# corywalker/llm_inference

Hardware: AMD Instinct MI355X
Metric: decode tokens/sec + achieved HBM GB/s vs roofline, Gemma-3 4B Q4_0 (higher is better)
Workload: dtype q4_0 x q8_0 int8 dot, fp32 accumulate; f16 logits table; 1 GPU; gemma-3-4b-q4_0 greedy decode after a 512-token prefill (BASELINE configs[2]); mode=fast, parallelism=single

## Files before the change

include/llmi.h:

```cpp
#ifndef LLMI_H
#define LLMI_H

#include <stddef.h>
#include <stdint.h>

#ifdef __cplusplus
extern "C" {
#endif

typedef enum {
  LLMI_OK = 0,
  LLMI_E_SIZE = 1,
  LLMI_E_TYPE = 2,
  LLMI_E_ARG = 3,
  LLMI_E_HIP = 4,
  LLMI_E_GGUF = 5,
  LLMI_E_NODEV = 6,
  LLMI_E_RANGE = 7
} llmi_status;

#define LLMI_EXACT 1u
#define LLMI_NO_GRAPH 2u
#define LLMI_TP_PEER 4u
#define LLMI_EXACT_KQ 8u
// ... 113 lines not shown

int llmi_session_enqueue(llmi_session* s, int32_t first, int pos, int n_steps);
int llmi_session_sync(llmi_session* s, int32_t* out_tokens, int n);

typedef struct {
  int n_layer, n_embd, n_ff, n_head, n_head_kv, head_dim, vocab, max_ctx;
  size_t weight_bytes;
  size_t bytes_per_token;
  size_t kv_bytes_per_pos;
  int kernels_per_token;
  int tp_rank, tp_size;
  int batched_prefill;
  int screened_logits;
  size_t screen_bytes;
  int prefill_f16_redo;
  int layer_engine;
  int ffn_engine;
  int tp_exchange;
  long long block_slow_waits;
  int exact_engine;
  int exact_batched_prefill;
  int prefill_gemm;
  int sampling;
  int score_path;
} llmi_session_info;
#define LLMI_SESSION_INFO_N_SEQ_OFFSET 132
#define LLMI_SESSION_INFO_N_SEQ(info) (*(const int*)((const char*)(info) + LLMI_SESSION_INFO_N_SEQ_OFFSET))
int llmi_session_get_info_sized(const llmi_session* s, llmi_session_info* info, size_t info_size);
int llmi_session_get_info(const llmi_session* s, llmi_session_info* info);
#define llmi_session_get_info(s, info) llmi_session_get_info_sized((s), (info), sizeof(llmi_session_info))

int llmi_session_time_kernel(llmi_session* s, int which, int reps, double* us_per_launch, double* bytes_per_launch);

int llmi_selftest(int which, unsigned long long* out);

#ifdef __cplusplus
}
#endif
#endif
```

llm_inference_amd/_lib.py:

```python
from __future__ import annotations

import ctypes as C
import os

import numpy as np

HERE = os.path.dirname(os.path.abspath(__file__))
LIB_PATH = os.environ.get("LLMI_LIB") or os.path.join(HERE, "libllmi.so")

LLMI_EXACT = 1
LLMI_NO_GRAPH = 2
LLMI_TP_PEER = 4
LLMI_EXACT_KQ = 8
PEER_HANDLE_BYTES = 64

STATUS = {0: "OK", 1: "E_SIZE", 2: "E_TYPE", 3: "E_ARG", 4: "E_HIP", 5: "E_GGUF", 6: "E_NODEV", 7: "E_RANGE"}


class LLMIError(RuntimeError):

    def __init__(self, code: int, msg: str):
        super().__init__(msg)
        self.code = code
        self.status = STATUS.get(code, str(code))
# ... 78 lines not shown
    "llmi_session_create":(C.c_int, [_vp, _sz, C.POINTER(SessionOpts), C.POINTER(_vp)]),
    "llmi_session_destroy": (None, [_vp]),
    "llmi_tp_unique_id": (C.c_int, [_vp]),
    "llmi_tp_group_create": (C.c_int, [C.c_int, C.POINTER(_vp)]),
    "llmi_tp_group_destroy": (None, [_vp]),
    "llmi_session_peer_handle": (C.c_int, [_vp, _vp]),
    "llmi_session_peer_connect": (C.c_int, [_vp, _vp]),
    "llmi_session_forward": (C.c_int, [_vp, _vp, C.c_int, C.c_int, _vp, _vp]),
    "llmi_session_score": (C.c_int, [_vp, _vp, C.c_int, C.c_int, _vp, _vp, _vp, _vp]),
    "llmi_session_seq_reserve": (C.c_int, [_vp, C.c_int]),
    "llmi_session_seq_copy": (C.c_int, [_vp, C.c_int, C.c_int, C.c_int]),
    "llmi_session_batch_forward": (C.c_int, [_vp, _vp, _vp, _vp, C.c_int, _vp, _vp, _vp]),
    "llmi_session_batch_extend": (C.c_int, [_vp, _vp, C.POINTER(Span), C.c_int, _vp, _vp, _vp]),
    "llmi_session_batch_generate": (C.c_int, [_vp, _vp, _vp, _vp, C.c_int, C.c_int, _vp, C.c_int, _vp]),
    "llmi_session_batch_generate_sampled": (C.c_int, [_vp, _vp, _vp, _vp, C.c_int, C.c_int, _vp, C.c_int,
                                                      C.POINTER(Sampler), _vp]),
    "llmi_session_batch_generate_lookup": (C.c_int, [_vp, _vp, _vp, _vp, _vp, C.c_int, C.POINTER(Lookup), C.c_int, _vp,
                                                     C.c_int, _vp, _vp, C.POINTER(LookupStats)]),
    "llmi_lookup_draft": (C.c_int, [_vp, C.c_int, C.c_int, C.c_int, C.c_int, _vp, C.POINTER(C.c_int),
                                    C.POINTER(C.c_int), C.POINTER(C.c_int)]),
    "llmi_logits_rows": (C.c_int, [_vp, _vp, C.c_int, C.c_int, C.c_int, _f32, _vp]),
    "llmi_logits_rows_rb": (C.c_int, [C.c_int]),
    "llmi_score_rows": (C.c_int, [_vp, _vp, C.c_int, C.c_int, C.c_int, _f32, _vp, _vp, _vp, _vp]),
    "llmi_session_generate": (C.c_int, [_vp, _i32, C.c_int, C.c_int, _vp]),
    "llmi_session_dump": (C.c_int, [_vp, _vp, C.c_int, C.c_int, C.c_char_p]),
    "llmi_session_enqueue": (C.c_int, [_vp, _i32, C.c_int, C.c_int]),
    "llmi_session_trace": (C.c_int, [_vp, _vp, C.c_int, C.c_int, _u32, _vp, _vp]),
    "llmi_session_sync": (C.c_int, [_vp, _vp, C.c_int]),
    "llmi_session_set_sampler": (C.c_int, [_vp, C.POINTER(Sampler)]),
    "llmi_sample_logits": (C.c_int, [_vp, _sz, C.POINTER(Sampler), C.c_int, _vp, _vp, _vp, _vp, _vp]),
    "llmi_session_get_info": (C.c_int, [_vp, _vp]),
    "llmi_session_get_info_sized": (C.c_int, [_vp, C.POINTER(SessionInfo), _sz]),
    "llmi_session_time_kernel": (C.c_int, [_vp, C.c_int, C.c_int, C.POINTER(_f64), C.POINTER(_f64)]),
    "llmi_selftest": (C.c_int, [C.c_int, _vp]),
}


def lib() -> C.CDLL:
    global _lib
    if _lib is None:
        if not os.path.exists(LIB_PATH):
            raise ImportError(f"{LIB_PATH} missing: build it with `python -m llm_inference_amd.build` "
                              "(HIP, --offload-arch=gfx950); there is no CPU fallback")
        L = C.CDLL(LIB_PATH)
        for name, (res, args) in _SIGS.items():
            f = getattr(L, name)
            f.restype = res
            f.argtypes = args
        _lib = L
    return _lib


def check(rc: int) -> None:
    if rc != 0:
        raise LLMIError(rc, lib().llmi_last_error().decode(errors="replace"))


def ptr(a: np.ndarray) -> int:
    return a.ctypes.data
```

llm_inference_amd/csrc/capi.cpp:

```cpp
#include <algorithm>
#include <cmath>
#include <cstddef>
#include <cstring>
#include <mutex>
#include <vector>

#include "score_plan.h"
#include "session.h"

using namespace llmi;

namespace {

thread_local std::string g_err;

struct Ctx {
  int device = -1;
  hipStream_t stream = nullptr;
  hipEvent_t ev_in = nullptr, ev_out = nullptr;
  std::vector<std::pair<void*, size_t>> bufs;
  void* get(int slot, size_t bytes) {
    if ((int)bufs.size() <= slot) bufs.resize(slot + 1, {nullptr, 0});
    auto& b = bufs[slot];
    if (b.second < bytes) {
// ... 701 lines not shown
      out[1] = r[1];
    } else if (which == 2) {
      size_t live = 0, cached = 0, grave = 0;
      dev_mem_stats(&live, &cached, &grave);
      out[0] = live;
      out[1] = cached;
      out[2] = grave;
    } else {
      throw status_error(LLMI_E_ARG, "selftest: unknown test");
    }
  });
}

int llmi_session_get_info_sized(const llmi_session* s, llmi_session_info* info, size_t info_size) {
  return guard([&] {
    if (!s || !info) throw status_error(LLMI_E_ARG, "get_info: null pointer");
    llmi_session_info full;
    std::memset(&full, 0, sizeof(full));
    s->s->info(&full);
    static_assert(sizeof(llmi_session_info) == LLMI_SESSION_INFO_N_SEQ_OFFSET + sizeof(int) &&
                      offsetof(llmi_session_info, score_path) + sizeof(int) == LLMI_SESSION_INFO_N_SEQ_OFFSET,
                  "n_seq lies in llmi_session_info's tail padding");
    const int n_seq = s->s->n_seq();
    std::memcpy(reinterpret_cast<char*>(&full) + LLMI_SESSION_INFO_N_SEQ_OFFSET, &n_seq, sizeof(int));
    std::memcpy(info, &full, std::min(info_size, sizeof(full)));
  });
}

static_assert(offsetof(llmi_session_info, score_path) == 128, "the struct's layout before score_path was appended");
int (llmi_session_get_info)(const llmi_session* s, llmi_session_info* info) {
  return llmi_session_get_info_sized(s, info, offsetof(llmi_session_info, score_path));
}

int llmi_session_time_kernel(llmi_session* s, int which, int reps, double* us, double* bytes) {
  return guard([&] { s->s->time_kernel(which, reps, us, bytes); });
}

}
```

llm_inference_amd/csrc/k_logits.hip:

```cpp
#include "session_kernels.h"

namespace llmi {

namespace {

__device__ __forceinline__ float dot8_h(uint4 w, uint4 x, float acc) {
  typedef _Float16 h2t __attribute__((ext_vector_type(2)));
  acc = __builtin_amdgcn_fdot2(__builtin_bit_cast(h2t, w.x), __builtin_bit_cast(h2t, x.x), acc, false);
  acc = __builtin_amdgcn_fdot2(__builtin_bit_cast(h2t, w.y), __builtin_bit_cast(h2t, x.y), acc, false);
  acc = __builtin_amdgcn_fdot2(__builtin_bit_cast(h2t, w.z), __builtin_bit_cast(h2t, x.z), acc, false);
  acc = __builtin_amdgcn_fdot2(__builtin_bit_cast(h2t, w.w), __builtin_bit_cast(h2t, x.w), acc, false);
  return acc;
}

__device__ __forceinline__ unsigned fkey(float f) {
  const unsigned u = __float_as_uint(f);
  return (u & 0x80000000u) ? ~u : (u | 0x80000000u);
}
__device__ __forceinline__ float fkey_inv(unsigned k) {
  return __uint_as_float((k & 0x80000000u) ? (k & 0x7FFFFFFFu) : ~k);
}

__global__ void quantize_table_q8_kernel(const uint16_t* __restrict__ w, size_t n_blocks, int nb,
                                         uint4* __restrict__ qs, uint16_t* __restrict__ d) {
  const size_t i = blockIdx.x * (size_t)blockDim.x + threadIdx.x;
  if (i >= n_blocks) return;
  const uint4* src = reinterpret_cast<const uint4*>(w + i * 32);
  float v[32];
#pragma unroll
  for (int k = 0; k < 4; k++) {
    const uint4 u = src[k];
    const uint32_t ws[4] = {u.x, u.y, u.z, u.w};
#pragma unroll
    for (int j = 0; j < 4; j++) {
      v[k * 8 + 2 * j] = h2f((uint16_t)(ws[j] & 0xFFFF));
      v[k * 8 + 2 * j + 1] = h2f((uint16_t)(ws[j] >> 16));
    }
  }
  float amax = 0.0f;
#pragma unroll
  for (int k = 0; k < 32; k++) amax = fmaxf(amax, fabsf(v[k]));
  const float want = amax / 127.0f;
  uint16_t dh = f2h_ggml(want);
  if (h2f(dh) < want) dh = (uint16_t)(dh + 1);
  const float df = h2f(dh);
  uint32_t packed[8];
#pragma unroll
  for (int k = 0; k < 8; k++) {
    uint32_t p = 0;
#pragma unroll
    for (int j = 0; j < 4; j++) {
      const int q = df > 0.0f ? (int)fminf(127.0f, fmaxf(-127.0f, rintf(v[4 * k + j] / df))) : 0;
      p |= (uint32_t)(q & 0xFF) << (8 * j);
    }
    packed[k] = p;
  }
  qs[2 * i] = make_uint4(packed[0], packed[1], packed[2], packed[3]);
  qs[2 * i + 1] = make_uint4(packed[4], packed[5], packed[6], packed[7]);
  d[i] = dh;
  (void)nb;
}

__global__ __launch_bounds__(1024) void screen_prep_kernel(const uint16_t* __restrict__ x16, int n, ScreenX* __restrict__ xs,
                                                           unsigned* __restrict__ m_key) {
  __shared__ double s_l1[256];
  const int t = threadIdx.x, b = t >> 2, sub = t & 3, nb = n / 32;
  if (b < nb) {
    float v[8];
#pragma unroll
    for (int i = 0; i < 8; i++) v[i] = h2f(x16[b * 32 + sub * 8 + i]);
    const double l1 = screen_prep_quad(v, sub, n, xs + b);
    if (sub == 0) s_l1[b] = l1;
  }
  __syncthreads();
  if (t < 64) screen_prep_total(s_l1, nb, xs, m_key);
}

template <int CPL, int AHEAD, int LPR = 32>
__global__ __launch_bounds__(256) void screen_gemv_kernel(const uint4* __restrict__ qs, const uint16_t* __restrict__ d,
                                                          int rows, int nb, const ScreenX* __restrict__ xs,
                                                          float* __restrict__ hi, unsigned* __restrict__ m_key) {
  static_assert(LPR == 32 || LPR == 16, "lanes per row");
  constexpr int RPW = 64 / LPR;
  const int NC = 2 * nb;
  const int lane = threadIdx.x & 63, j = lane % LPR, sub = lane / LPR;
  int grp = blockIdx.x * 4 + (threadIdx.x >> 6);
  const int ngrp = gridDim.x * 4;
  int4 xq[CPL];
  float xd[CPL], xc[CPL];
#pragma unroll
  for (int p = 0; p < CPL; p++) {
    const int c = p * LPR + j, b = min(c, NC - 1) >> 1;
    const bool ok = c < NC;
    const int4* xb = reinterpret_cast<const int4*>(xs + b);
    xq[p] = ok ? ((c & 1) ? xb[1] : xb[0]) : make_int4(0, 0, 0, 0);
    xd[p] = ok ? xs[b].dx : 0.0f;
    xc[p] = ok ? xs[b].c_half : 0.0f;
  }
  const float A = xs[nb].a;
  float mloc = -INFINITY;
  auto load = [&](uint4 (&q)[CPL], uint16_t (&s)[CPL], int r) {
    const uint4* qr = qs + (size_t)r * NC;
    const uint16_t* dr = d + (size_t)r * nb;
#pragma unroll
    for (int p = 0; p < CPL; p++) {
      const int c = min(p * LPR + j, NC - 1);
      q[p] = ld_nt(qr + c);
      s[p] = dr[c >> 1];
    }
  };
  auto row_sum = [](float v) { return LPR == 32 ? half_sum(v) : row16_sum(v); };
  int row = RPW * grp + sub;
  uint4 cq[CPL];
  uint16_t cs[CPL];
  load(cq, cs, min(row, rows - 1));
  uint4 mq[AHEAD > 1 ? CPL : 1];
  uint16_t ms[AHEAD > 1 ? CPL : 1];
  if constexpr (AHEAD > 1) load(mq, ms, min(row + RPW * ngrp, rows - 1));
  for (; RPW * grp < rows; grp += ngrp, row += RPW * ngrp) {
    uint4 nq[CPL];
    uint16_t ns[CPL];
    load(nq, ns, min(row + RPW * AHEAD * ngrp, rows - 1));
    float ap = 0.0f, bp = 0.0f;
#pragma unroll
    for (int p = 0; p < CPL; p++) {
      int is = 0;
      is = sdot4((int)cq[p].x, xq[p].x, is);
      is = sdot4((int)cq[p].y, xq[p].y, is);
      is = sdot4((int)cq[p].z, xq[p].z, is);
      is = sdot4((int)cq[p].w, xq[p].w, is);
      const float dw = h2f(cs[p]);
      ap += dw * (xd[p] * (float)is);
      bp += dw * xc[p];
    }
    ap = row_sum(ap);
    bp = row_sum(bp) * (1.0f + 0x1p-10f);
    if (j == 0 && row < rows) {
      hi[row] = (ap + bp) + A;
      mloc = fmaxf(mloc, (ap - bp) - A);
    }
#pragma unroll
    for (int p = 0; p < CPL; p++) {
      if constexpr (AHEAD > 1) {
        cq[p] = mq[p];
        cs[p] = ms[p];
        mq[p] = nq[p];
        ms[p] = ns[p];
      } else {
        cq[p] = nq[p];
        cs[p] = ns[p];
      }
    }
  }
  mloc = wave_max(mloc);
  if (lane == 0 && mloc > -INFINITY) atomicMax(m_key, fkey(mloc));
}

template <int P, int T>
__global__ __launch_bounds__(256) void screen_rescore_kernel(const uint4* __restrict__ w, int rows,
                                                             const uint4* __restrict__ x16, const float* __restrict__ hi,
                                                             const unsigned* __restrict__ m_key, int slice,
                                                             unsigned long long* __restrict__ amax_key) {
  constexpr int NP = P + (T ? 1 : 0);
  constexpr int RU4 = P * 64 + T;
  extern __shared__ int s_cand[];
  __shared__ int s_n;
  const int t = threadIdx.x, lane = t & 63, wave = t >> 6;
  if (t == 0) s_n = 0;
  __syncthreads();
  const float M = fkey_inv(*m_key);
  const int r0 = blockIdx.x * slice, r1 = min(rows, r0 + slice);
  for (int r = r0 + t; r < r1; r += 256)
    if (hi[r] >= M) s_cand[atomicAdd(&s_n, 1)] = r;
  __syncthreads();
  const int n = s_n;
  if (n == 0) return;
  const int tl = T ? lane % (T ? T : 64) : lane;
  uint4 xr[NP];
#pragma unroll
  for (int p = 0; p < NP; p++) xr[p] = x16[p * 64 + (p < P ? lane : tl)];
  unsigned long long best = 0;
  for (int k = wave; k < n; k += 4) {
    const int row = s_cand[k];
    const uint4* wr = w + (size_t)row * RU4;
    uint4 cur[NP];
#pragma unroll
    for (int p = 0; p < NP; p++) cur[p] = ld_nt(wr + p * 64 + (p < P ? lane : tl));
    float acc = 0.0f;
#pragma unroll
    for (int p = 0; p < P; p++) acc = dot8_h(cur[p], xr[p], acc);
    if constexpr (T != 0) {
      const float tt = dot8_h(cur[P], xr[P], 0.0f);
      acc += lane < T ? tt : 0.0f;
    }
    acc = wave_sum(acc);
    const unsigned long long key = argmax_key(acc, (uint32_t)row);
    best = key > best ? key : best;
  }
  if (lane == 0 && best) atomicMax(amax_key, best);
}

__global__ __launch_bounds__(256) void screen_rescore_exact_kernel(const uint16_t* __restrict__ w, int rows, int cols,
                                                                   const uint16_t* __restrict__ x16,
                                                                   const float* __restrict__ hi,
                                                                   const unsigned* __restrict__ m_key, int slice,
                                                                   unsigned long long* __restrict__ amax_key) {
  extern __shared__ int s_cand[];
  __shared__ int s_n;
  const int t = threadIdx.x;
  if (t == 0) s_n = 0;
  __syncthreads();
  const float M = fkey_inv(*m_key);
  const int r0 = blockIdx.x * slice, r1 = min(rows, r0 + slice);
  for (int r = r0 + t; r < r1; r += 256)
    if (hi[r] >= M) s_cand[atomicAdd(&s_n, 1)] = r;
  __syncthreads();
  const int n = s_n;
  const int np = cols & ~31, l = t & 3;
  unsigned long long best = 0;
  for (int c0 = 0; c0 < n; c0 += 64) {
    const int ci = c0 + (t >> 2);
    const bool ok = ci < n;
    const int row = ok ? s_cand[ci] : s_cand[0];
    const uint16_t* wr = w + (size_t)row * cols;
    float acc[8] = {0, 0, 0, 0, 0, 0, 0, 0};
    for (int k0 = 0; k0 < np; k0 += 32 * 16) {
      uint4 wv[16], xv[16];
#pragma unroll
      for (int u = 0; u < 16; u++) {
        const int k = min(k0 + 32 * u, np - 32);
        wv[u] = *reinterpret_cast<const uint4*>(wr + k + 8 * l);
        xv[u] = *reinterpret_cast<const uint4*>(x16 + k + 8 * l);
      }
#pragma unroll
      for (int u = 0; u < 16; u++) {
        if (k0 + 32 * u >= np) break;
        const uint32_t ww[4] = {wv[u].x, wv[u].y, wv[u].z, wv[u].w}, xx[4] = {xv[u].x, xv[u].y, xv[u].z, xv[u].w};
#pragma unroll
        for (int e = 0; e < 4; e++) {
          acc[2 * e] = fmaf(h2f((uint16_t)(ww[e] & 0xFFFF)), h2f((uint16_t)(xx[e] & 0xFFFF)), acc[2 * e]);
          acc[2 * e + 1] = fmaf(h2f((uint16_t)(ww[e] >> 16)), h2f((uint16_t)(xx[e] >> 16)), acc[2 * e + 1]);
        }
      }
    }
    float v[8];
#pragma unroll
    for (int m = 0; m < 8; m++) {
      const float a = acc[m] + __shfl_xor(acc[m], 1);
      v[m] = a + __shfl_xor(a, 2);
    }
    if (ok && l == 0) {
      const float t0 = v[0] + v[4], t1 = v[1] + v[5], t2 = v[2] + v[6], t3 = v[3] + v[7];
      float r = (t0 + t1) + (t2 + t3);
      for (int k = np; k < cols; k++) r = fmaf(h2f(wr[k]), h2f(x16[k]), r);
      const unsigned long long key = argmax_key(r, (uint32_t)row);
      best = key > best ? key : best;
    }
  }
  if (best) atomicMax(amax_key, best);
}

constexpr int RESCORE_SLICE = 1024;

}

bool screen_supported(const DevWeight& table) {
  return table.type == T_F16 && table.cols % 128 == 0 && table.cols >= 128 && table.cols <= 6144 && table.rows > 0;
}

void alloc_screen_table(const DevWeight& table, ScreenTable& st, hipStream_t s) {
  const int nb = table.cols / 32;
  const size_t n_blocks = (size_t)table.rows * nb;
  st.qs = static_cast<decltype(st.qs)>(dev_alloc(n_blocks * 32));
  st.d = static_cast<decltype(st.d)>(dev_alloc(n_blocks * 2 + 64));
  st.xs = static_cast<decltype(st.xs)>(dev_alloc((size_t)(nb + 1) * sizeof(ScreenX)));
  st.hi = static_cast<decltype(st.hi)>(dev_alloc((size_t)table.rows * 4));
  st.m_key = static_cast<decltype(st.m_key)>(dev_alloc(64));
  LLMI_HIP(hipMemsetAsync(st.xs, 0, (size_t)(nb + 1) * sizeof(ScreenX), s));
  LLMI_HIP(hipMemsetAsync(st.m_key, 0, 64, s));
  st.rows = table.rows;
  st.cols = table.cols;
  st.bytes = n_blocks * 34;
  hipLaunchKernelGGL(quantize_table_q8_kernel, dim3((unsigned)((n_blocks + 255) / 256)), dim3(256), 0, s,
                     reinterpret_cast<const uint16_t*>(table.qs), n_blocks, nb, reinterpret_cast<uint4*>(st.qs), st.d);
  LLMI_HIP(hipGetLastError());
}

void free_screen_table(ScreenTable& st) {
  for (void* p : {(void*)st.qs, (void*)st.d, (void*)st.xs, (void*)st.hi, (void*)st.m_key})
    dev_free(p);
  st = ScreenTable{};
}

void launch_screen_argmax(const DevWeight& table, const ScreenTable& st, const uint16_t* x16,
                          unsigned long long* amax_key, hipStream_t s, bool prepped, bool exact) {
  if (table.rows != st.rows || table.cols != st.cols) throw std::runtime_error("screen: table mismatch");
  if (!screen_supported(table)) throw std::runtime_error("screen: unsupported logits table");
  const int n = table.cols, nb = n / 32;
  if (nb > 256) throw std::runtime_error("screen: n_embd > 8192");
  if (!prepped) hipLaunchKernelGGL(screen_prep_kernel, dim3(1), dim3(1024), 0, s, x16, n, st.xs, st.m_key);
  const int rows = table.rows;
  constexpr int wpc = 8;
  constexpr int ahead = 2;
  const int lpr = 2 * nb <= 80 ? 16 : 32;
  const int cpl = (2 * nb + lpr - 1) / lpr, rpw = 64 / lpr;
  const dim3 grid((std::min((rows + rpw - 1) / rpw, 256 * wpc) + 3) / 4);
  auto go = [&](auto kern) {
    hipLaunchKernelGGL(kern, grid, dim3(256), 0, s, reinterpret_cast<const uint4*>(st.qs), st.d, rows, nb, st.xs, st.hi,
                       st.m_key);
  };
  switch (cpl) {
#define LLMI_SCR(C)                                                       \
  case C:                                                                 \
    if (lpr == 16) go(ahead > 1 ? screen_gemv_kernel<C, 2, 16> : screen_gemv_kernel<C, 1, 16>); \
    else go(ahead > 1 ? screen_gemv_kernel<C, 2, 32> : screen_gemv_kernel<C, 1, 32>);           \
    break;
    LLMI_SCR(1) LLMI_SCR(2) LLMI_SCR(3) LLMI_SCR(4) LLMI_SCR(5) LLMI_SCR(6) LLMI_SCR(7) LLMI_SCR(8) LLMI_SCR(9)
    LLMI_SCR(10) LLMI_SCR(11) LLMI_SCR(12)
#undef LLMI_SCR
    default: throw std::runtime_error("screen: unsupported n_embd");
  }
  LLMI_HIP(hipGetLastError());
  const int u4 = n / 8, P = u4 / 64, T = u4 % 64;
  const dim3 rg((rows + RESCORE_SLICE - 1) / RESCORE_SLICE);
  const size_t lds = RESCORE_SLICE * sizeof(int);
  if (exact) {
    hipLaunchKernelGGL(screen_rescore_exact_kernel, rg, dim3(256), lds, s, reinterpret_cast<const uint16_t*>(table.qs),
                       rows, n, x16, st.hi, st.m_key, RESCORE_SLICE, amax_key);
    LLMI_HIP(hipGetLastError());
    return;
  }
  switch (P * 4 + T / 16) {
#define LLMI_RSC(PP, TT)                                                                                          \
  case PP * 4 + TT / 16:                                                                                          \
    hipLaunchKernelGGL((screen_rescore_kernel<PP, TT>), rg, dim3(256), lds, s,                                   \
                       reinterpret_cast<const uint4*>(table.qs), rows, reinterpret_cast<const uint4*>(x16), st.hi, \
                       st.m_key, RESCORE_SLICE, amax_key);                                                        \
    break;
#define LLMI_RSC4(PP) LLMI_RSC(PP, 0) LLMI_RSC(PP, 16) LLMI_RSC(PP, 32) LLMI_RSC(PP, 48)
    LLMI_RSC(0, 16) LLMI_RSC(0, 32) LLMI_RSC(0, 48) LLMI_RSC4(1) LLMI_RSC4(2) LLMI_RSC4(3) LLMI_RSC4(4) LLMI_RSC4(5)
    LLMI_RSC4(6) LLMI_RSC4(7) LLMI_RSC4(8) LLMI_RSC4(9) LLMI_RSC4(10) LLMI_RSC4(11) LLMI_RSC(12, 0)
#undef LLMI_RSC4
#undef LLMI_RSC
    default: throw std::runtime_error("screen: unsupported logits width for the rescoring kernel");
  }
  LLMI_HIP(hipGetLastError());
}

}
```

llm_inference_amd/csrc/session.cpp:

```cpp
#include "session.h"
#include "score_plan.h"

#include <cmath>
#include <functional>
#include <cstdio>
#include <cstring>

namespace llmi {

static int meta_u32(const GGUFView& g, const std::string& k, bool required, int dflt = 0) {
  const GValue* v = g.find(k);
  if (!v) {
    if (required) throw status_error(LLMI_E_GGUF, "Failed to find metadata key: " + k);
    return dflt;
  }
  return (int)v->u32;
}

void Session::load_hparams(const GGUFView& g) {
  const GValue* a = g.find("general.architecture");
  if (!a) throw status_error(LLMI_E_GGUF, "Failed to find metadata key: general.architecture");
  hp_.arch = a->str;
  const std::string p = hp_.arch + ".";
  hp_.n_layer = meta_u32(g, p + "block_count", true);
// ... 2015 lines not shown
    throw status_error(LLMI_E_HIP, (e == 2 ? std::string("tensor-parallel push exchange: a received slice failed its "
                                                         "checksum (device results invalid)")
                                           : std::string("tensor-parallel push exchange: a peer's slice did not arrive "
                                                         "within LLMI_PX_TIMEOUT_MS (device results invalid)")) +
                                       coll_->fail_detail());
  }
  if (blk_trace_) {
    std::vector<unsigned long long> h(4096 * 8);
    LLMI_HIP(hipMemcpy(h.data(), blk_trace_, h.size() * 8, hipMemcpyDeviceToHost));
    if (const char* path = getenv("LLMI_BLOCK_TRACE_OUT"))
      if (FILE* f = fopen(path, "ab")) {
        fwrite(h.data(), 8, h.size(), f);
        fclose(f);
      }
  }
  if (!blk_err_) return;
  int ev[2] = {0, 0};
  LLMI_HIP(hipMemcpyAsync(ev, blk_err_, sizeof(ev), hipMemcpyDeviceToHost, stream_));
  LLMI_HIP(hipStreamSynchronize(stream_));
  const int e = ev[0];
  if (ev[1]) {
    slow_waits_ += ev[1];
    LLMI_HIP(hipMemsetAsync(blk_err_ + 1, 0, sizeof(int), stream_));
    LLMI_HIP(hipStreamSynchronize(stream_));
  }
  if (e) {
    LLMI_HIP(hipMemsetAsync(blk_err_, 0, sizeof(int), stream_));
    LLMI_HIP(hipMemsetAsync(ticket_, 0, sizeof(unsigned) * (size_t)hp_.n_head, stream_));
    LLMI_HIP(hipStreamSynchronize(stream_));
    throw status_error(LLMI_E_HIP, "attention block: a cross-work-group wait timed out (device results invalid)");
  }
}

void Session::info(llmi_session_info* o) const {
  o->n_layer = hp_.n_layer;
  o->n_embd = hp_.n_embd;
  o->n_ff = hp_.n_ff;
  o->n_head = hp_.n_head;
  o->n_head_kv = hp_.n_head_kv;
  o->head_dim = hp_.hd_k;
  o->vocab = vocab_;
  o->max_ctx = max_ctx_;
  o->weight_bytes = weight_bytes_;
  o->tp_rank = tp_rank_;
  o->tp_size = tp_size_;
  o->batched_prefill = prefill_ok_ ? 1 : 0;
  o->screened_logits = screen_ ? 1 : 0;
  o->screen_bytes = screen_ ? scr_.bytes : 0;
  o->prefill_f16_redo = pf_f16_redo_;
  o->layer_engine = 0;
  o->ffn_engine = 0;
  o->tp_exchange = coll_ ? (px_fused_ && coll_->kind() == EX_PUSH ? EX_PUSH_FUSED : coll_->kind()) : 0;
  o->block_slow_waits = slow_waits_;
  o->exact_engine = xl_ ? 1 : 0;
  o->exact_batched_prefill = xp_ok() ? 1 : 0;
  o->prefill_gemm = !prefill_ok_ ? 0 : prefill_f16_ok() ? (pf_kq_ ? 6 : 7) : 5;
  size_t b = logits_w_.bytes;
  for (const auto& l : L_) {
    for (const auto& p : l.qkv) b += p.w.bytes;
    for (const auto& p : l.gate_up) b += p.w.bytes;
    b += l.o.w.bytes + l.down.w.bytes;
  }
  o->bytes_per_token = b;
  size_t kv = 0;
  for (const auto& l : L_) kv += (size_t)2 * nkv_ * l.hd * 2;
  o->kv_bytes_per_pos = kv;
// ... 237 lines not shown
```

llm_inference_amd/csrc/session.h:

```cpp
#pragma once

#include <cstdio>
#include <memory>
#include <string>
#include <utility>
#include <vector>

#include "../../include/llmi.h"
#include "collective.h"
#include "exact.h"
#include "gguf_reader.h"
#include "sample.h"
#include "session_kernels.h"

namespace llmi {

struct status_error : std::runtime_error {
  int code;
  status_error(int c, const std::string& m) : std::runtime_error(m), code(c) {}
};

void validate_sampler(const llmi_sampler& sp);

struct HParams {
// ... 39 lines not shown
};

class Session {
 public:
  Session(const uint8_t* gguf, size_t size, const llmi_session_opts& opts);
  ~Session();
  Session(const Session&) = delete;
  Session& operator=(const Session&) = delete;

  void forward(const int32_t* tokens, int n_tokens, int pos, float* logits, int32_t* argmax);
  void forward_dump(const int32_t* tokens, int n_tokens, int pos, const char* path);
  void forward_trace(const int32_t* tokens, int n_tokens, int pos, bool gen, llmi_trace_fn fn, void* user,
                     bool score = false);
  void score(const int32_t* tokens, int n_tokens, int pos, const int32_t* targets, float* logprob, float* lse,
             int32_t* argmax);
  void seq_reserve(int n_seq);
  int n_seq() const { return n_seq_; }
  void seq_copy(int dst, int src, int n_pos);
  void batch_forward(const int32_t* tokens, const int32_t* slots, const int32_t* pos, int B, float* logits,
                     int32_t* argmax, float* lse);
  void batch_generate(const int32_t* first, const int32_t* slots, const int32_t* pos, int B, int n_steps,
                      const int32_t* stop, int n_stop, int32_t* out);
  void batch_extend(const int32_t* tokens, const llmi_span* spans, int n_spans, float* logits, int32_t* argmax,
                    float* lse);
  void batch_generate_lookup(const int32_t* hist, const int32_t* hist_len, const int32_t* slots, const int32_t* pos,
                             int B, const llmi_lookup& lk, int max_steps, const int32_t* stop, int n_stop, int32_t* out,
                             int32_t* n_out, llmi_lookup_stats* stats);
  void batch_generate_sampled(const int32_t* first, const int32_t* slots, const int32_t* pos, int B, int n_steps,
                              const int32_t* stop, int n_stop, const llmi_sampler* samplers, int32_t* out);
  void enqueue(int32_t first, int pos, int n_steps);
  void sync(int32_t* out_tokens, int n);
  void set_sampler(const llmi_sampler* sp);
  void info(llmi_session_info* out) const;
  void time_kernel(int which, int reps, double* us, double* bytes);
  void peer_handle(void* out) const;
  void peer_connect(const void* handles);

 private:
  void release();
  void load_hparams(const GGUFView& g);
  void setup_tp();
  void upload(const GGUFView& g);
  void alloc_buffers();
  void build_rope_tables();
  void record_step(hipStream_t s, bool gen = false, bool fold_embed = false, bool logits = true, bool sample = false);
  bool embed_fold_ok() const;
  bool sample_fold_ok() const;
  NormOut embed_out() const;
  bool down_plain(const LayerDev& Ld) const;
  void record_logits(hipStream_t s, bool gen = false);
  void prefill(const int32_t* tokens, int n, int pos);
  bool prefill_f16_ok() const;
  bool prefill_run(const int32_t* tokens, int n, int pos, bool allow_f16);
  void prefill_layers(const int32_t* d_tokens, int T, int p0, bool trim, bool last_chunk, bool f16_all,
                      const SeqRow* rows, const AttnBlock* blocks = nullptr, int n_blocks = 0);
  void gather_cols(void* buf, size_t pitch_b, size_t slice_b, int T, hipStream_t s);
  void ensure_prefill_buffers(int cap);
  void record_layers(hipStream_t s, bool x_q8);
  void record_layers_fused(hipStream_t s, bool x_q8);
  bool xl_ = false;
  bool exact_kq_ = false;
  double* xa_scores_ = nullptr;
  XBlock* xa_xq_ = nullptr;
  void setup_xl();
  void record_layers_xl(hipStream_t s);
  bool xp_ok() const;
// ... 205 lines not shown
```

llm_inference_amd/csrc/session_kernels.h:

```cpp
#pragma once

#include "attn.h"
#include "kernels.h"
#include "px.h"

namespace llmi {

size_t gguf_bytes(uint32_t type, size_t rows, size_t cols);
bool gemv_type_supported(uint32_t type);
DevWeight alloc_weight(uint32_t type, int rows, int cols, size_t slack = 64);
void upload_rows(DevWeight& w, int dst_row0, const void* host, int rows, hipStream_t s);
void free_weight(DevWeight& w);
void* dev_alloc(size_t bytes);
void dev_free(void* p);
void session_live(int delta);
void session_constructed(bool ok);
void dev_mem_stats(size_t* live, size_t* cached, size_t* grave);
void to_slab_layout(DevWeight& w, hipStream_t s);
void to_kq_layout(DevWeight& w, hipStream_t s, int slab = 0);

struct ScreenX;
struct NormOut {
  float* xn = nullptr;
  XBlock* q8 = nullptr;
// ... 135 lines not shown
  int32_t id[4];
  int n;
};
void launch_batch_feedback(const int32_t* argmax, SeqRow* rows, int32_t* tokens, int B, BatchStops stops, int32_t* out,
                           hipStream_t s);
constexpr int PREFILL_ATTN_KS_MAX = 8;
void launch_prefill_norm(const PrefillNorm& a, int T, hipStream_t s);
bool prefill_gemm_supported(const DevWeight& w);
void launch_prefill_gemm(const DevWeight& w, const XBlock* x, int xstride, int T, float* out, int ostride,
                         hipStream_t s);
bool prefill_gemm16_supported(const DevWeight& w);
bool prefill_gemm7_supported(const DevWeight& w);
void launch_prefill_gemm16(const DevWeight& w, const uint16_t* x, int xstride, int T, float* out, int ostride,
                           const float* tscale, hipStream_t s);
void launch_prefill_qk(const PrefillQK& a, int T, hipStream_t s);
void launch_prefill_attn(const PrefillAttn& a, int T, hipStream_t s);
void launch_prefill_gelu(const float* gu, int F, int H, XBlock* xq, int xstride, int T, hipStream_t s,
                         uint16_t* x16 = nullptr, int x16stride = 0, int q8k = 0, float* tscale = nullptr);

int layer_gemv_slab(const DevWeight& w, int role);
int layer_gemv_gelu_group(int cols, uint32_t type = T_Q4_0);
int launch_layer_gemv(const DevWeight& w, LayerGemv a, int role, hipStream_t s);
bool layer_gemv2_supported(const DevWeight& wa, const DevWeight& wb, int role);
void launch_layer_gemv2(const DevWeight& wa, const DevWeight& wb, LayerGemv a, int role, hipStream_t s);
void launch_quantize_q8k_xblocks(const float* x, int n, XBlock* xb, hipStream_t s);
void launch_argmax(const float* x, int n, unsigned long long* key, hipStream_t s);
struct ScreenX {
  int4 lo, hi;
  float dx, c_half, a, pad;
};
static_assert(sizeof(ScreenX) == 48, "ScreenX layout");
struct ScreenTable {
  uint8_t* qs = nullptr;
  uint16_t* d = nullptr;
  ScreenX* xs = nullptr;
  float* hi = nullptr;
  unsigned* m_key = nullptr;
  int rows = 0, cols = 0;
  size_t bytes = 0;
};
bool screen_supported(const DevWeight& table);
void alloc_screen_table(const DevWeight& table, ScreenTable& st, hipStream_t s);
void free_screen_table(ScreenTable& st);
void launch_screen_argmax(const DevWeight& table, const ScreenTable& st, const uint16_t* x16,
                          unsigned long long* amax_key, hipStream_t s, bool prepped = false, bool exact = false);

constexpr float SCREEN_DENORM = 6.103515625e-05f;
__device__ __forceinline__ double screen_prep_quad(const float (&v)[8], int sub, int n, ScreenX* __restrict__ o) {
  float amax = 0.0f;
#pragma unroll
  for (int i = 0; i < 8; i++) amax = fmaxf(amax, fabsf(v[i]));
  amax = fmaxf(amax, __shfl_xor(amax, 1));
  amax = fmaxf(amax, __shfl_xor(amax, 2));
  const float dx = amax / 127.0f;
  double l1 = 0.0, e = 0.0, den = 0.0;
  uint32_t packed[2] = {0, 0};
#pragma unroll
  for (int i = 0; i < 8; i++) {
    const int q = dx > 0.0f ? (int)fminf(127.0f, fmaxf(-127.0f, rintf(v[i] / dx))) : 0;
    packed[i / 4] |= (uint32_t)(q & 0xFF) << (8 * (i % 4));
    l1 += fabs((double)v[i]);
    e += fabs((double)v[i] - (double)dx * (double)q);
    if (fabsf(v[i]) < SCREEN_DENORM) den += fabs((double)v[i]);
  }
#pragma unroll
  for (int m = 1; m <= 2; m <<= 1) {
    l1 += __shfl_xor(l1, m);
    e += __shfl_xor(e, m);
    den += __shfl_xor(den, m);
  }
  int* words = reinterpret_cast<int*>(o);
// ... 29 lines not shown
```

llm_inference_amd/model.py:

```python
from __future__ import annotations

import ctypes as C
from dataclasses import dataclass
from typing import NamedTuple, Optional, Sequence

import numpy as np

from ._lib import (BATCH_TOKENS_MAX, LLMI_EXACT, LLMI_EXACT_KQ, LLMI_NO_GRAPH, LLMI_TP_PEER, PEER_HANDLE_BYTES, SPAN_ALL,
                   SPAN_LAST, SPAN_NONE, TP_ID_BYTES, TRACE_FN, Lookup, LookupStats, Sampler, SessionInfo, SessionOpts,
                   Span, check, lib, ptr)
from .gguf import GGUFFile
from .score import ScoreResult, resolve_targets


def tp_unique_id() -> bytes:
    b = C.create_string_buffer(TP_ID_BYTES)
    check(lib().llmi_tp_unique_id(b))
    return b.raw


class TPGroup:

    def __init__(self, size: int):
        h = C.c_void_p()
# ... 299 lines not shown
        lk = Lookup(int(draft_len), int(ngram_max), int(ngram_min), int(max_new))
        stats = LookupStats()
        check(lib().llmi_session_batch_generate_lookup(self.h, ptr(tokens) if tokens.size else None, ptr(hl), ptr(sl),
                                                       ptr(p), B, C.byref(lk), int(max_steps),
                                                       ptr(st) if st.size else None, st.size, ptr(out), ptr(n_out),
                                                       C.byref(stats)))
        return LookupResult([out[b, :n_out[b]].copy() for b in range(B)], int(stats.steps),
                            np.array(stats.drafted[:B], np.int32), np.array(stats.accepted[:B], np.int32))

    def enqueue(self, first: int, pos: int, n_steps: int) -> None:
        check(lib().llmi_session_enqueue(self.h, first, pos, n_steps))

    def sync(self, n: int = 0) -> Optional[np.ndarray]:
        out = np.zeros(max(n, 1), np.int32)
        check(lib().llmi_session_sync(self.h, ptr(out) if n else None, n))
        return out[:n] if n else None

    def peer_handle(self) -> bytes:
        b = C.create_string_buffer(PEER_HANDLE_BYTES)
        check(lib().llmi_session_peer_handle(self.h, b))
        return b.raw

    def peer_connect(self, handles: Sequence[bytes]) -> None:
        if len(handles) != self.info.tp_size or any(len(h) != PEER_HANDLE_BYTES for h in handles):
            raise ValueError(f"need {self.info.tp_size} handles of {PEER_HANDLE_BYTES} bytes")
        b = C.create_string_buffer(b"".join(handles), PEER_HANDLE_BYTES * len(handles))
        check(lib().llmi_session_peer_connect(self.h, b))

    def time_kernel(self, which: int, reps: int):
        us, by = C.c_double(), C.c_double()
        check(lib().llmi_session_time_kernel(self.h, which, reps, C.byref(us), C.byref(by)))
        return us.value, by.value

    def close(self):
        if getattr(self, "h", None):
            lib().llmi_session_destroy(self.h)
            self.h = None

    def __del__(self):
        self.close()
```

Before: 903.8 tokens/s.

## Group screen-table scales per 128 columns and pack them for vector loads

The int8 logits screen table now stores one f16 scale per group of columns (default 128, set by LLMI_SCREEN_GROUP) instead of one per 32-element block. The scales are laid out per lane slot so each lane loads its scales as a few uint4 non-temporal loads rather than one scattered uint16 load per block. The screen GEMV prefetch is rebuilt as a ring of AHEAD+1 register buffers instead of rotating copies, and wpc/ahead become runtime knobs read from environment variables. A candidate counter is added to the rescore kernels and exposed through a new API for diagnostics. Coarser scales cut scale traffic but loosen the screening bound, which may let more rows through to the exact rescore.

```diff
diff --git a/include/llmi.h b/include/llmi.h
--- a/include/llmi.h
+++ b/include/llmi.h
@@ -169,6 +169,8 @@
 
 int llmi_session_time_kernel(llmi_session* s, int which, int reps, double* us_per_launch, double* bytes_per_launch);
 
+int llmi_session_screen_candidates(llmi_session* s, long long* rows);
+
 int llmi_selftest(int which, unsigned long long* out);
 
 #ifdef __cplusplus
diff --git a/llm_inference_amd/_lib.py b/llm_inference_amd/_lib.py
--- a/llm_inference_amd/_lib.py
+++ b/llm_inference_amd/_lib.py
@@ -134,6 +134,7 @@
     "llmi_session_get_info": (C.c_int, [_vp, _vp]),
     "llmi_session_get_info_sized": (C.c_int, [_vp, C.POINTER(SessionInfo), _sz]),
     "llmi_session_time_kernel": (C.c_int, [_vp, C.c_int, C.c_int, C.POINTER(_f64), C.POINTER(_f64)]),
+    "llmi_session_screen_candidates": (C.c_int, [_vp, C.POINTER(C.c_longlong)]),
     "llmi_selftest": (C.c_int, [C.c_int, _vp]),
 }
 
diff --git a/llm_inference_amd/csrc/capi.cpp b/llm_inference_amd/csrc/capi.cpp
--- a/llm_inference_amd/csrc/capi.cpp
+++ b/llm_inference_amd/csrc/capi.cpp
@@ -757,6 +757,13 @@
   return llmi_session_get_info_sized(s, info, offsetof(llmi_session_info, score_path));
 }
 
+int llmi_session_screen_candidates(llmi_session* s, long long* rows) {
+  return guard([&] {
+    if (!s || !rows) throw status_error(LLMI_E_ARG, "screen_candidates: null pointer");
+    *rows = s->s->screen_candidates();
+  });
+}
+
 int llmi_session_time_kernel(llmi_session* s, int which, int reps, double* us, double* bytes) {
   return guard([&] { s->s->time_kernel(which, reps, us, bytes); });
 }
diff --git a/llm_inference_amd/csrc/k_logits.hip b/llm_inference_amd/csrc/k_logits.hip
--- a/llm_inference_amd/csrc/k_logits.hip
+++ b/llm_inference_amd/csrc/k_logits.hip
@@ -21,12 +21,8 @@
   return __uint_as_float((k & 0x80000000u) ? (k & 0x7FFFFFFFu) : ~k);
 }
 
-__global__ void quantize_table_q8_kernel(const uint16_t* __restrict__ w, size_t n_blocks, int nb,
-                                         uint4* __restrict__ qs, uint16_t* __restrict__ d) {
-  const size_t i = blockIdx.x * (size_t)blockDim.x + threadIdx.x;
-  if (i >= n_blocks) return;
-  const uint4* src = reinterpret_cast<const uint4*>(w + i * 32);
-  float v[32];
+__device__ __forceinline__ void load_block32(const uint16_t* __restrict__ w, float (&v)[32]) {
+  const uint4* src = reinterpret_cast<const uint4*>(w);
 #pragma unroll
   for (int k = 0; k < 4; k++) {
     const uint4 u = src[k];
@@ -37,28 +33,43 @@
       v[k * 8 + 2 * j + 1] = h2f((uint16_t)(ws[j] >> 16));
     }
   }
+}
+__global__ void quantize_table_q8_kernel(const uint16_t* __restrict__ w, size_t n_groups, int nb, int ng, int gb, int S,
+                                         int ns, uint4* __restrict__ qs, uint16_t* __restrict__ d) {
+  const size_t i = blockIdx.x * (size_t)blockDim.x + threadIdx.x;
+  if (i >= n_groups) return;
+  const size_t row = i / (size_t)ng;
+  const int g = (int)(i - row * (size_t)ng);
+  const int b0 = g * gb, b1 = min(nb, b0 + gb);
+  const size_t blk0 = row * (size_t)nb;
+  float v[32];
   float amax = 0.0f;
-#pragma unroll
-  for (int k = 0; k < 32; k++) amax = fmaxf(amax, fabsf(v[k]));
+  for (int b = b0; b < b1; b++) {
+    load_block32(w + (blk0 + b) * 32, v);
+#pragma unroll
+    for (int k = 0; k < 32; k++) amax = fmaxf(amax, fabsf(v[k]));
+  }
   const float want = amax / 127.0f;
   uint16_t dh = f2h_ggml(want);
   if (h2f(dh) < want) dh = (uint16_t)(dh + 1);
   const float df = h2f(dh);
-  uint32_t packed[8];
-#pragma unroll
-  for (int k = 0; k < 8; k++) {
-    uint32_t p = 0;
-#pragma unroll
-    for (int j = 0; j < 4; j++) {
-      const int q = df > 0.0f ? (int)fminf(127.0f, fmaxf(-127.0f, rintf(v[4 * k + j] / df))) : 0;
-      p |= (uint32_t)(q & 0xFF) << (8 * j);
-    }
-    packed[k] = p;
-  }
-  qs[2 * i] = make_uint4(packed[0], packed[1], packed[2], packed[3]);
-  qs[2 * i + 1] = make_uint4(packed[4], packed[5], packed[6], packed[7]);
-  d[i] = dh;
-  (void)nb;
+  for (int b = b0; b < b1; b++) {
+    load_block32(w + (blk0 + b) * 32, v);
+    uint32_t packed[8];
+#pragma unroll
+    for (int k = 0; k < 8; k++) {
+      uint32_t p = 0;
+#pragma unroll
+      for (int j = 0; j < 4; j++) {
+        const int q = df > 0.0f ? (int)fminf(127.0f, fmaxf(-127.0f, rintf(v[4 * k + j] / df))) : 0;
+        p |= (uint32_t)(q & 0xFF) << (8 * j);
+      }
+      packed[k] = p;
+    }
+    qs[2 * (blk0 + b)] = make_uint4(packed[0], packed[1], packed[2], packed[3]);
+    qs[2 * (blk0 + b) + 1] = make_uint4(packed[4], packed[5], packed[6], packed[7]);
+  }
+  d[((row * S + g % S) * ns) * 8 + g / S] = dh;
 }
 
 __global__ __launch_bounds__(1024) void screen_prep_kernel(const uint16_t* __restrict__ x16, int n, ScreenX* __restrict__ xs,
@@ -76,14 +87,20 @@
   if (t < 64) screen_prep_total(s_l1, nb, xs, m_key);
 }
 
+__device__ __forceinline__ float scale_f16(const uint4& u, int k) {
+  const uint32_t w = k < 2 ? u.x : k < 4 ? u.y : k < 6 ? u.z : u.w;
+  return h2f((uint16_t)((k & 1) ? w >> 16 : w & 0xFFFFu));
+}
 template <int CPL, int AHEAD, int LPR = 32>
-__global__ __launch_bounds__(256) void screen_gemv_kernel(const uint4* __restrict__ qs, const uint16_t* __restrict__ d,
-                                                          int rows, int nb, const ScreenX* __restrict__ xs,
+__global__ __launch_bounds__(256) void screen_gemv_kernel(const uint4* __restrict__ qs, const uint4* __restrict__ ds,
+                                                          int rows, int nb, int gsh, const ScreenX* __restrict__ xs,
                                                           float* __restrict__ hi, unsigned* __restrict__ m_key) {
   static_assert(LPR == 32 || LPR == 16, "lanes per row");
   constexpr int RPW = 64 / LPR;
+  constexpr int NS = (CPL + 7) / 8;
   const int NC = 2 * nb;
   const int lane = threadIdx.x & 63, j = lane % LPR, sub = lane / LPR;
+  const int S = LPR >> gsh, slot = j >> gsh;
   int grp = blockIdx.x * 4 + (threadIdx.x >> 6);
   const int ngrp = gridDim.x * 4;
   int4 xq[CPL];
@@ -99,28 +116,24 @@
   }
   const float A = xs[nb].a;
   float mloc = -INFINITY;
-  auto load = [&](uint4 (&q)[CPL], uint16_t (&s)[CPL], int r) {
+  auto load = [&](uint4 (&q)[CPL], uint4 (&s)[NS], int r) {
     const uint4* qr = qs + (size_t)r * NC;
-    const uint16_t* dr = d + (size_t)r * nb;
+    const uint4* dr = ds + ((size_t)r * S + slot) * NS;
+#pragma unroll
+    for (int k = 0; k < NS; k++) s[k] = ld_nt(dr + k);
 #pragma unroll
     for (int p = 0; p < CPL; p++) {
       const int c = min(p * LPR + j, NC - 1);
       q[p] = ld_nt(qr + c);
-      s[p] = dr[c >> 1];
     }
   };
   auto row_sum = [](float v) { return LPR == 32 ? half_sum(v) : row16_sum(v); };
   int row = RPW * grp + sub;
-  uint4 cq[CPL];
-  uint16_t cs[CPL];
-  load(cq, cs, min(row, rows - 1));
-  uint4 mq[AHEAD > 1 ? CPL : 1];
-  uint16_t ms[AHEAD > 1 ? CPL : 1];
-  if constexpr (AHEAD > 1) load(mq, ms, min(row + RPW * ngrp, rows - 1));
-  for (; RPW * grp < rows; grp += ngrp, row += RPW * ngrp) {
-    uint4 nq[CPL];
-    uint16_t ns[CPL];
-    load(nq, ns, min(row + RPW * AHEAD * ngrp, rows - 1));
+  constexpr int NBUF = AHEAD + 1;
+  uint4 bq[NBUF][CPL], bs[NBUF][NS];
+#pragma unroll
+  for (int k = 0; k < NBUF; k++) load(bq[k], bs[k], min(row + k * RPW * ngrp, rows - 1));
+  auto step = [&](uint4 (&cq)[CPL], uint4 (&cs)[NS]) {
     float ap = 0.0f, bp = 0.0f;
 #pragma unroll
     for (int p = 0; p < CPL; p++) {
@@ -129,27 +142,28 @@
       is = sdot4((int)cq[p].y, xq[p].y, is);
       is = sdot4((int)cq[p].z, xq[p].z, is);
       is = sdot4((int)cq[p].w, xq[p].w, is);
-      const float dw = h2f(cs[p]);
+      const float dw = scale_f16(cs[p / 8], p % 8);
       ap += dw * (xd[p] * (float)is);
       bp += dw * xc[p];
     }
+    load(cq, cs, min(row + RPW * NBUF * ngrp, rows - 1));
     ap = row_sum(ap);
     bp = row_sum(bp) * (1.0f + 0x1p-10f);
     if (j == 0 && row < rows) {
       hi[row] = (ap + bp) + A;
       mloc = fmaxf(mloc, (ap - bp) - A);
     }
-#pragma unroll
-    for (int p = 0; p < CPL; p++) {
-      if constexpr (AHEAD > 1) {
-        cq[p] = mq[p];
-        cs[p] = ms[p];
-        mq[p] = nq[p];
-        ms[p] = ns[p];
-      } else {
-        cq[p] = nq[p];
-        cs[p] = ns[p];
+    grp += ngrp;
+    row += RPW * ngrp;
+  };
+  for (bool more = true; more;) {
+#pragma unroll
+    for (int k = 0; k < NBUF; k++) {
+      if (RPW * grp >= rows) {
+        more = false;
+        break;
       }
+      step(bq[k], bs[k]);
     }
   }
   mloc = wave_max(mloc);
@@ -160,7 +174,8 @@
 __global__ __launch_bounds__(256) void screen_rescore_kernel(const uint4* __restrict__ w, int rows,
                                                              const uint4* __restrict__ x16, const float* __restrict__ hi,
                                                              const unsigned* __restrict__ m_key, int slice,
-                                                             unsigned long long* __restrict__ amax_key) {
+                                                             unsigned long long* __restrict__ amax_key,
+                                                             unsigned long long* __restrict__ n_cand) {
   constexpr int NP = P + (T ? 1 : 0);
   constexpr int RU4 = P * 64 + T;
   extern __shared__ int s_cand[];
@@ -175,6 +190,7 @@
   __syncthreads();
   const int n = s_n;
   if (n == 0) return;
+  if (t == 0) atomicAdd(n_cand, (unsigned long long)n);
   const int tl = T ? lane % (T ? T : 64) : lane;
   uint4 xr[NP];
 #pragma unroll
@@ -204,7 +220,8 @@
                                                                    const uint16_t* __restrict__ x16,
                                                                    const float* __restrict__ hi,
                                                                    const unsigned* __restrict__ m_key, int slice,
-                                                                   unsigned long long* __restrict__ amax_key) {
+                                                                   unsigned long long* __restrict__ amax_key,
+                                                                   unsigned long long* __restrict__ n_cand) {
   extern __shared__ int s_cand[];
   __shared__ int s_n;
   const int t = threadIdx.x;
@@ -216,6 +233,7 @@
     if (hi[r] >= M) s_cand[atomicAdd(&s_n, 1)] = r;
   __syncthreads();
   const int n = s_n;
+  if (t == 0 && n) atomicAdd(n_cand, (unsigned long long)n);
   const int np = cols & ~31, l = t & 3;
   unsigned long long best = 0;
   for (int c0 = 0; c0 < n; c0 += 64) {
@@ -268,26 +286,49 @@
   return table.type == T_F16 && table.cols % 128 == 0 && table.cols >= 128 && table.cols <= 6144 && table.rows > 0;
 }
 
+namespace {
+int screen_lpr(int nb) { return 2 * nb <= 80 ? 16 : 32; }
+int screen_knob(const char* name, int dflt) {
+  const char* e = getenv(name);
+  return e && *e ? atoi(e) : dflt;
+}
+}
+
 void alloc_screen_table(const DevWeight& table, ScreenTable& st, hipStream_t s) {
   const int nb = table.cols / 32;
   const size_t n_blocks = (size_t)table.rows * nb;
+  const int lpr = screen_lpr(nb), cpl = (2 * nb + lpr - 1) / lpr;
+  const int group = screen_knob("LLMI_SCREEN_GROUP", 128);
+  if (group < 32 || (group & (group - 1)) || group / 16 > lpr) throw std::runtime_error("screen: unsupported scale group");
+  st.group = group;
+  st.slots = lpr / (group / 16);
+  st.slot_u4 = (cpl + 7) / 8;
+  st.wpc = std::min(32, std::max(1, screen_knob("LLMI_SCREEN_WPC", 8)));
+  st.ahead = screen_knob("LLMI_SCREEN_AHEAD", 2) > 1 ? 2 : 1;
+  const int gb = group / 32, ng = (nb + gb - 1) / gb;
+  const size_t n_groups = (size_t)table.rows * ng;
+  const size_t d_bytes = (size_t)table.rows * st.slots * st.slot_u4 * 16;
   st.qs = static_cast<decltype(st.qs)>(dev_alloc(n_blocks * 32));
-  st.d = static_cast<decltype(st.d)>(dev_alloc(n_blocks * 2 + 64));
+  st.d = static_cast<decltype(st.d)>(dev_alloc(d_bytes + 64));
   st.xs = static_cast<decltype(st.xs)>(dev_alloc((size_t)(nb + 1) * sizeof(ScreenX)));
   st.hi = static_cast<decltype(st.hi)>(dev_alloc((size_t)table.rows * 4));
   st.m_key = static_cast<decltype(st.m_key)>(dev_alloc(64));
+  st.n_cand = static_cast<decltype(st.n_cand)>(dev_alloc(64));
   LLMI_HIP(hipMemsetAsync(st.xs, 0, (size_t)(nb + 1) * sizeof(ScreenX), s));
   LLMI_HIP(hipMemsetAsync(st.m_key, 0, 64, s));
+  LLMI_HIP(hipMemsetAsync(st.n_cand, 0, 64, s));
+  LLMI_HIP(hipMemsetAsync(st.d, 0, d_bytes + 64, s));
   st.rows = table.rows;
   st.cols = table.cols;
-  st.bytes = n_blocks * 34;
-  hipLaunchKernelGGL(quantize_table_q8_kernel, dim3((unsigned)((n_blocks + 255) / 256)), dim3(256), 0, s,
-                     reinterpret_cast<const uint16_t*>(table.qs), n_blocks, nb, reinterpret_cast<uint4*>(st.qs), st.d);
+  st.bytes = n_blocks * 32 + d_bytes;
+  hipLaunchKernelGGL(quantize_table_q8_kernel, dim3((unsigned)((n_groups + 255) / 256)), dim3(256), 0, s,
+                     reinterpret_cast<const uint16_t*>(table.qs), n_groups, nb, ng, gb, st.slots, st.slot_u4,
+                     reinterpret_cast<uint4*>(st.qs), reinterpret_cast<uint16_t*>(st.d));
   LLMI_HIP(hipGetLastError());
 }
 
 void free_screen_table(ScreenTable& st) {
-  for (void* p : {(void*)st.qs, (void*)st.d, (void*)st.xs, (void*)st.hi, (void*)st.m_key})
+  for (void* p : {(void*)st.qs, (void*)st.d, (void*)st.xs, (void*)st.hi, (void*)st.m_key, (void*)st.n_cand})
     dev_free(p);
   st = ScreenTable{};
 }
@@ -300,14 +341,16 @@
   if (nb > 256) throw std::runtime_error("screen: n_embd > 8192");
   if (!prepped) hipLaunchKernelGGL(screen_prep_kernel, dim3(1), dim3(1024), 0, s, x16, n, st.xs, st.m_key);
   const int rows = table.rows;
-  constexpr int wpc = 8;
-  constexpr int ahead = 2;
-  const int lpr = 2 * nb <= 80 ? 16 : 32;
+  const int wpc = st.wpc, ahead = st.ahead;
+  const int lpr = screen_lpr(nb);
   const int cpl = (2 * nb + lpr - 1) / lpr, rpw = 64 / lpr;
+  int gsh = 0;
+  while ((16 << gsh) < st.group) gsh++;
+  if ((lpr >> gsh) != st.slots || (cpl + 7) / 8 != st.slot_u4) throw std::runtime_error("screen: scale layout mismatch");
   const dim3 grid((std::min((rows + rpw - 1) / rpw, 256 * wpc) + 3) / 4);
   auto go = [&](auto kern) {
-    hipLaunchKernelGGL(kern, grid, dim3(256), 0, s, reinterpret_cast<const uint4*>(st.qs), st.d, rows, nb, st.xs, st.hi,
-                       st.m_key);
+    hipLaunchKernelGGL(kern, grid, dim3(256), 0, s, reinterpret_cast<const uint4*>(st.qs), st.d, rows, nb, gsh, st.xs,
+                       st.hi, st.m_key);
   };
   switch (cpl) {
 #define LLMI_SCR(C)                                                       \
@@ -326,7 +369,7 @@
   const size_t lds = RESCORE_SLICE * sizeof(int);
   if (exact) {
     hipLaunchKernelGGL(screen_rescore_exact_kernel, rg, dim3(256), lds, s, reinterpret_cast<const uint16_t*>(table.qs),
-                       rows, n, x16, st.hi, st.m_key, RESCORE_SLICE, amax_key);
+                       rows, n, x16, st.hi, st.m_key, RESCORE_SLICE, amax_key, st.n_cand);
     LLMI_HIP(hipGetLastError());
     return;
   }
@@ -335,7 +378,7 @@
   case PP * 4 + TT / 16:                                                                                          \
     hipLaunchKernelGGL((screen_rescore_kernel<PP, TT>), rg, dim3(256), lds, s,                                   \
                        reinterpret_cast<const uint4*>(table.qs), rows, reinterpret_cast<const uint4*>(x16), st.hi, \
-                       st.m_key, RESCORE_SLICE, amax_key);                                                        \
+                       st.m_key, RESCORE_SLICE, amax_key, st.n_cand);                                             \
     break;
 #define LLMI_RSC4(PP) LLMI_RSC(PP, 0) LLMI_RSC(PP, 16) LLMI_RSC(PP, 32) LLMI_RSC(PP, 48)
     LLMI_RSC(0, 16) LLMI_RSC(0, 32) LLMI_RSC(0, 48) LLMI_RSC4(1) LLMI_RSC4(2) LLMI_RSC4(3) LLMI_RSC4(4) LLMI_RSC4(5)
diff --git a/llm_inference_amd/csrc/session.cpp b/llm_inference_amd/csrc/session.cpp
--- a/llm_inference_amd/csrc/session.cpp
+++ b/llm_inference_amd/csrc/session.cpp
@@ -2071,6 +2071,14 @@
   }
 }
 
+long long Session::screen_candidates() {
+  if (!screen_) return 0;
+  unsigned long long v = 0;
+  LLMI_HIP(hipStreamSynchronize(stream_));
+  LLMI_HIP(hipMemcpy(&v, scr_.n_cand, sizeof(v), hipMemcpyDeviceToHost));
+  return (long long)v;
+}
+
 void Session::info(llmi_session_info* o) const {
   o->n_layer = hp_.n_layer;
   o->n_embd = hp_.n_embd;
diff --git a/llm_inference_amd/csrc/session.h b/llm_inference_amd/csrc/session.h
--- a/llm_inference_amd/csrc/session.h
+++ b/llm_inference_amd/csrc/session.h
@@ -95,6 +95,7 @@
   void sync(int32_t* out_tokens, int n);
   void set_sampler(const llmi_sampler* sp);
   void info(llmi_session_info* out) const;
+  long long screen_candidates();
   void time_kernel(int which, int reps, double* us, double* bytes);
   void peer_handle(void* out) const;
   void peer_connect(const void* handles);
diff --git a/llm_inference_amd/csrc/session_kernels.h b/llm_inference_amd/csrc/session_kernels.h
--- a/llm_inference_amd/csrc/session_kernels.h
+++ b/llm_inference_amd/csrc/session_kernels.h
@@ -191,11 +191,14 @@
 static_assert(sizeof(ScreenX) == 48, "ScreenX layout");
 struct ScreenTable {
   uint8_t* qs = nullptr;
-  uint16_t* d = nullptr;
+  uint4* d = nullptr;
   ScreenX* xs = nullptr;
   float* hi = nullptr;
   unsigned* m_key = nullptr;
+  unsigned long long* n_cand = nullptr;
   int rows = 0, cols = 0;
+  int group = 0, slots = 0, slot_u4 = 0;
+  int wpc = 0, ahead = 0;
   size_t bytes = 0;
 };
 bool screen_supported(const DevWeight& table);
diff --git a/llm_inference_amd/model.py b/llm_inference_amd/model.py
--- a/llm_inference_amd/model.py
+++ b/llm_inference_amd/model.py
@@ -355,6 +355,11 @@
         check(lib().llmi_session_time_kernel(self.h, which, reps, C.byref(us), C.byref(by)))
         return us.value, by.value
 
+    def screen_candidates(self) -> int:
+        n = C.c_longlong()
+        check(lib().llmi_session_screen_candidates(self.h, C.byref(n)))
+        return n.value
+
     def close(self):
         if getattr(self, "h", None):
             lib().llmi_session_destroy(self.h)
diff --git a/llm_inference_amd/screen_ref.py b/llm_inference_amd/screen_ref.py
--- /dev/null
+++ b/llm_inference_amd/screen_ref.py
@@ -0,0 +1,59 @@
+import numpy as np
+
+SCREEN_DENORM = np.float32(2.0 ** -14)
+WIDEN = 1.0 + 2.0 ** -10
+
+
+def _round_up_f32(v: np.ndarray) -> np.ndarray:
+    f = v.astype(np.float32)
+    return np.where(f.astype(np.float64) < v, np.nextafter(f, np.float32(np.inf)), f).astype(np.float32)
+
+
+def quantize_table(w16: np.ndarray, group: int):
+    V, n = w16.shape
+    ng = (n + group - 1) // group
+    w = w16.astype(np.float32)
+    pad = ng * group - n
+    wp = np.pad(w, ((0, 0), (0, pad))) if pad else w
+    amax = np.abs(wp).reshape(V, ng, group).max(axis=2)
+    want = amax / np.float32(127.0)
+    d = want.astype(np.float16)
+    low = d.astype(np.float32) < want
+    d = np.where(low, (d.view(np.uint16) + np.uint16(1)).view(np.float16), d)
+    df = np.repeat(d.astype(np.float32), group, axis=1)[:, :n]
+    with np.errstate(divide="ignore", invalid="ignore"):
+        q = np.where(df > 0, np.clip(np.rint(w / df), -127, 127), 0).astype(np.int8)
+    return q, d
+
+
+def prep_x(x16: np.ndarray):
+    n = x16.shape[0]
+    nb = n // 32
+    v = x16.astype(np.float32).reshape(nb, 32)
+    dx = (np.abs(v).max(axis=1) / np.float32(127.0)).astype(np.float32)
+    with np.errstate(divide="ignore", invalid="ignore"):
+        q = np.where(dx[:, None] > 0, np.clip(np.rint(v / dx[:, None]), -127, 127), 0).astype(np.int8)
+    v64 = v.astype(np.float64)
+    l1 = np.abs(v64).sum(axis=1)
+    e = np.abs(v64 - dx.astype(np.float64)[:, None] * q).sum(axis=1)
+    den = np.where(np.abs(v) < SCREEN_DENORM, np.abs(v64), 0.0).sum(axis=1)
+    k_u = (n + 32) * 2.0 ** -24
+    c = (0.5 * l1 + 127.5 * e + 127.5 * k_u * (l1 + e) + 127.5 * den) * WIDEN
+    c = 2.0 * _round_up_f32(0.5 * c).astype(np.float64)
+    A = _round_up_f32(np.array(2.0 * float(SCREEN_DENORM) * l1.sum() * WIDEN))
+    return q.reshape(n), dx, c.astype(np.float32), np.float32(A)
+
+
+def screen_rows(q: np.ndarray, d: np.ndarray, group: int, qx: np.ndarray, dx: np.ndarray, c: np.ndarray):
+    V, n = q.shape
+    nb = n // 32
+    isum = np.einsum("vbk,bk->vb", q.reshape(V, nb, 32).astype(np.int32), qx.reshape(nb, 32).astype(np.int32))
+    db = d.astype(np.float32)[:, np.arange(nb) * 32 // group]
+    approx = (db * (dx[None, :] * isum.astype(np.float32))).sum(axis=1, dtype=np.float32)
+    B = (db * c[None, :]).sum(axis=1, dtype=np.float32) * np.float32(WIDEN)
+    return approx, B
+
+
+def candidates(approx: np.ndarray, B: np.ndarray, A: np.float32) -> int:
+    M = (approx - B - A).max()
+    return int(((approx + B + A) >= M).sum())
```

Result: no change. 904.8 tokens/s, median of 4 (+0.1%).
